# JiaoXianjun/multi-rtl-sdr-calibration

Hardware: AMD Instinct MI355X
Metric: IQ Msamples/s through FCCH+SCH calib (higher is better)
Workload: dtype f64; 1 GPU; cfg4 full chain gsm_sync_demod.m:107-124: 64 dongle streams (64/GPU) x 1020000 IQ samples (102 frames), fir1(46), FCCH+SCH+total_ppm_calculation, table on the host; streams_per_gpu=64, streams_total=64, output=table, collective=none, rows_checked_vs_oracle_per_rank=0

## Files before the change

multi-rtl-sdr-calibration_amd/csrc/kernels_detect.h:

```cpp
#pragma once
#include "state.h"
#include "kernels_frontend.h"

__device__ __forceinline__ constexpr int fft16_rev(int k) { return ((k & 1) << 3) | ((k & 2) << 1) | ((k & 4) >> 1) | ((k & 8) >> 3); }
__device__ __forceinline__ void fft16(cplx* x) {
    const double c1 = 0.92387953251128673848, s1 = 0.38268343236508978178;
    const double r2 = 0.70710678118654752440;
    const cplx w16[8] = {{1.0, 0.0}, {c1, -s1}, {r2, -r2}, {s1, -c1}, {0.0, -1.0}, {-s1, -c1}, {-r2, -r2}, {-c1, -s1}};
#pragma unroll
    for (int len = 16; len >= 2; len >>= 1) {
        const int half = len >> 1, step = 16 / len;
#pragma unroll
        for (int i = 0; i < 16; i += len) {
#pragma unroll
            for (int j = 0; j < half; ++j) {
                const cplx u = x[i + j], v = x[i + j + half];
                x[i + j] = make_double2(u.x + v.x, u.y + v.y);
                const cplx d = make_double2(u.x - v.x, u.y - v.y);
                const int t = j * step;
                if (t == 0) x[i + j + half] = d;
                else if (t == 4) x[i + j + half] = make_double2(d.y, -d.x);
                else x[i + j + half] = cmul(d, w16[t]);
            }
        }
// ... 1246 lines not shown
    __shared__ double sh_e[FK_THREADS / 64];
    __shared__ float sh_m[FK_THREADS / 64];
    __shared__ int sh_cnt;
    __shared__ double sh_D;
    const int tid = threadIdx.x;
    const int nstep = nshift - 1;
    const int nchunk = (nstep + FS_CHUNK - 1) / FS_CHUNK;
    const int total = *n_items;
    fft37_tables(w37, wN2, N2, tid, tw_g);
    DEV_STAMP(KID_CHUNK, blockIdx.x, 0);
    for (int it = blockIdx.x; it < total; it += gridDim.x) {
    const int item = items[it];
    const int c = item & 0xFF, widx = item >> 8, s = widx / H, w = widx - s * H;
    const double pstar = cert && cert[widx].p > 0.0 ? cert[widx].p : 0.0;
    const int t0 = c * FS_CHUNK;
    const int lim = nstep - t0 < FS_CHUNK ? nstep - t0 : FS_CHUNK;
    const cplx* x = win + (size_t)s * win_stream_stride + (size_t)w * win_stride + t0;
    __syncthreads();
    for (int i = tid; i < nfft + lim; i += FK_THREADS) xs[i] = x[i];
    if (tid == 0) sh_cnt = 0;
    __syncthreads();
    double e = 0.0;
    for (int i = tid; i < nfft; i += FK_THREADS) e += fabs(xs[i].x) + fabs(xs[i].y);
    if (tid < FS_CHUNK) {
        float2 v = make_float2(0.0f, 0.0f);
        double dabs = 0.0;
        if (tid < lim) {
            const cplx a1 = xs[tid + nfft], b1 = xs[tid];
            const double dr = a1.x - b1.x, di = a1.y - b1.y;
            v = make_float2((float)dr, (float)di);
            dabs = fabs(dr) + fabs(di);
            e += dabs;
        }
        d[tid] = v;
        dabs = wave_sum(dabs);
        if (tid == 0) sh_D = dabs;
    }
    for (int off = 32; off > 0; off >>= 1) e += __shfl_down(e, off, 64);
    if ((tid & 63) == 0) sh_e[tid >> 6] = e;
    __syncthreads();
    fft37_step1_sym(xs, B, w37, tw_g, nfft, N2, ldb, tid, FK_THREADS);
    __syncthreads();
    double es = 0.0;
    for (int i = 0; i < FK_THREADS / 64; ++i) es += sh_e[i];
    const double E = FS_ERR_SCALE_CHUNK * es;
    const int npair = nfft >> 1;
    const double sp = sqrt(pstar);
    ChunkRec* r = rec + ((size_t)s * H + w) * nchunk + c;
    float m = 0.0f;
    for (int g0 = 0; g0 < npair; g0 += FK_THREADS) {
        const int g = g0 + tid;
        const bool act = g < npair;
        const int jj = g / 37, kr = g - jj * 37;
        const int k0 = kr + 37 * jj, k1 = jj == 0 ? kr + 37 * (N2 >> 1) : kr + 37 * (N2 - jj);
        v2f best = {0.0f, 0.0f};
        if (act) {
            cplx X0, X1;
            fft37_step2_pair(B, wN2, N2, ldb, kr, jj, &X0, &X1);
            const cplx t0w = tw_g[k0], t1w = tw_g[k1];
            const v2f wr = {(float)t0w.x, (float)t1w.x}, wi = {(float)-t0w.y, (float)-t1w.y};
            v2f xr = {(float)X0.x, (float)X1.x}, xi = {(float)X0.y, (float)X1.y};
            if (c == 0) best = xr * xr + xi * xi;
            const double D = sh_D * (1.0 + 1e-9);
            const bool sweep = !(pstar > 0.0) || !((sqrt(X0.x * X0.x + X0.y * X0.y) + D) * (1.0 + 1e-9) < sp) ||
                               !((sqrt(X1.x * X1.x + X1.y * X1.y) + D) * (1.0 + 1e-9) < sp);
            if (sweep) {
#pragma unroll 8
            for (int t = 0; t < FS_CHUNK; ++t) {
                const float2 dv = d[t];
                const v2f dr = {dv.x, dv.x}, di = {dv.y, dv.y};
                const v2f ar = xr + dr, ai = xi + di;
                xr = ar * wr - ai * wi;
                xi = ar * wi + ai * wr;
                const v2f p = xr * xr + xi * xi;
                best.x = fmaxf(best.x, p.x);
                best.y = fmaxf(best.y, p.y);
            }
            }
            if (k1 == k0) best.y = 0.0f;
            m = fmaxf(m, fmaxf(best.x, best.y));
        }
        float mm = m;
        for (int off = 32; off > 0; off >>= 1) mm = fmaxf(mm, __shfl_xor(mm, off, 64));
        __syncthreads();
        if ((tid & 63) == 0) sh_m[tid >> 6] = mm;
        __syncthreads();
        float bm = sh_m[0];
        for (int i = 1; i < FK_THREADS / 64; ++i) bm = fmaxf(bm, sh_m[i]);
        double thr = sqrt((double)bm) - E;
        if (sp > thr) thr = sp;
        thr = (thr - E) * (1.0 - 1e-6);
        if (act && sqrt((double)best.x) >= thr) {
            const int i = atomicAdd(&sh_cnt, 1);
            if (i < FK_CAP) { r->cand[i].k = k0; r->cand[i].p = best.x; }
        }
        if (act && k1 != k0 && sqrt((double)best.y) >= thr) {
            const int i = atomicAdd(&sh_cnt, 1);
            if (i < FK_CAP) { r->cand[i].k = k1; r->cand[i].p = best.y; }
        }
    }
    __syncthreads();
    for (int off = 32; off > 0; off >>= 1) m = fmaxf(m, __shfl_xor(m, off, 64));
    if ((tid & 63) == 0) sh_m[tid >> 6] = m;
    __syncthreads();
    if (tid == 0) {
        float bm = sh_m[0];
        for (int i = 1; i < FK_THREADS / 64; ++i) bm = fmaxf(bm, sh_m[i]);
        r->amax = bm;
        r->E = E;
        r->count = sh_cnt <= FK_CAP ? sh_cnt : -1;
    }
    DEV_STAMP(KID_CHUNK, blockIdx.x, 1 + (it / gridDim.x < 6 ? it / gridDim.x : 6));
    }
}

__global__ void k_fine_openall(const StreamState* __restrict__ sts, int nchunk, int H, int* __restrict__ items,
                               int* __restrict__ n_items) {
    const int s = blockIdx.y, w = blockIdx.x;
    if (w >= sts[s].n_win) return;
    __shared__ int base;
    if (threadIdx.x == 0) base = atomicAdd(n_items, nchunk);
    __syncthreads();
    for (int c = threadIdx.x; c < nchunk; c += blockDim.x) items[base + c] = ((s * H + w) << 8) | c;
}

#define FV_MAX_ITEMS 512
#define FV_THREADS 256
__device__ __forceinline__ void peak_store(PeakOut* dst, const PeakOut& o) {
    static_assert(sizeof(PeakOut) == 16, "two 64-bit words");
    unsigned long long* d = (unsigned long long*)dst;
    __hip_atomic_store(d, (unsigned long long)__double_as_longlong(o.p), __ATOMIC_RELAXED, __HIP_MEMORY_SCOPE_AGENT);
    __hip_atomic_store(d + 1, (unsigned long long)(unsigned)o.tie | ((unsigned long long)(unsigned)o.k << 32), __ATOMIC_RELAXED,
                       __HIP_MEMORY_SCOPE_AGENT);
}
template <int FVT, int ANB = 19>
__device__ __forceinline__ void fine_verify_body(const StreamState* __restrict__ sts,
                                                 const cplx* __restrict__ win, long win_stream_stride,
                                                 long win_stride, int nshift, int nfft,
                                                 const cplx* __restrict__ tw_g, const ChunkRec* __restrict__ rec,
                                                 PeakOut* __restrict__ out, int H,
                                                 const FineCert* __restrict__ cert, int* __restrict__ n_open,
                                                 unsigned char* smem, PeakOut* res = nullptr) {
    if (blockIdx.x == 0 && blockIdx.y == 0 && threadIdx.x == 0) *n_open = 0;
    const int wlen = nshift - 1 + nfft;
    cplx* xs = (cplx*)smem;
    cplx* anchor = xs + wlen;
    int* items = (int*)(anchor + FV_MAX_ITEMS);
    __shared__ int n_items, n_over;
    __shared__ double red_p[FVT / 64];
    __shared__ int red_t[FVT / 64], red_k[FVT / 64];
    const int s = blockIdx.y, w = blockIdx.x;
    if (w >= sts[s].n_win) return;
    const int tid = threadIdx.x, lane = tid & 63, wave = tid >> 6;
    const int nstep = nshift - 1;
    const int nchunk = (nstep + FS_CHUNK - 1) / FS_CHUNK;
    FineCert fc;
    fc.p = -1.0; fc.t = 0x7fffffff; fc.k = 0x7fffffff; fc.nch = nchunk; fc.nsuf = 0;
    if (cert) {
        fc = cert[(size_t)s * H + w];
        if (fc.nch == 0) {
            if (tid == 0) { PeakOut o2; o2.p = fc.p; o2.tie = fc.t; o2.k = fc.k; if (res) *res = o2; else peak_store(&out[(size_t)s * H + w], o2); }
            return;
        }
    }
    const int nopen = fc.nch, nsuf = fc.nsuf;
    ChunkRec* r = (ChunkRec*)smem;
    {
        const uint4* src = (const uint4*)(rec + ((size_t)s * H + w) * nchunk);
        uint4* dst = (uint4*)r;
        constexpr int Q = (int)(sizeof(ChunkRec) / 16);
        for (int i = tid; i < nopen * Q; i += FVT) { const int j = i / Q; dst[i] = src[fc_open_chunk(j, nopen, nsuf, nchunk) * Q + (i - j * Q)]; }
    }
    if (tid == 0) { n_items = 0; n_over = 0; }
    __syncthreads();
    double L = fc.p > 0.0 ? sqrt(fc.p) : 0.0;
    for (int c = 0; c < nopen; ++c) {
        const double v = sqrt((double)r[c].amax) - r[c].E;
        if (v > L) L = v;
    }
    L *= 1.0 - 1e-9;
    for (int i = tid; i < nopen * FK_CAP; i += FVT) {
        const int c = i / FK_CAP, q = i - c * FK_CAP;
        const int cnt = r[c].count;
        if (cnt < 0) { if (q == 0) atomicAdd(&n_over, 1); continue; }
        if (q >= cnt) continue;
        const ChunkCand cc = r[c].cand[q];
        if (sqrt((double)cc.p) + r[c].E >= L) {
            const int idx = atomicAdd(&n_items, 1);
            if (idx < FV_MAX_ITEMS) items[idx] = (cc.k << 8) | fc_open_chunk(c, nopen, nsuf, nchunk);
        }
    }
    __syncthreads();
    const bool slow = n_over > 0 || n_items > FV_MAX_ITEMS;
    DEV_STAMP(KID_VERIFY, blockIdx.y * gridDim.x + blockIdx.x, 3);
    if (n_items == 0 && !slow && fc.p > 0.0) {
        if (tid == 0) { PeakOut o2; o2.p = fc.p; o2.tie = fc.t; o2.k = fc.k; if (res) *res = o2; else peak_store(&out[(size_t)s * H + w], o2); }
        return;
    }
    const cplx* x = win + (size_t)s * win_stream_stride + (size_t)w * win_stride;
    double best = -1.0;
    int bt = 0x7fffffff, bk = 0x7fffffff;
    if (tid == 0 && fc.p > 0.0) { best = fc.p; bt = fc.t; bk = fc.k; }
    if (n_items > 0 || slow) {
        for (int i = tid; i < wlen; i += FVT) xs[i] = x[i];
        __syncthreads();
        const long total = slow ? (long)nopen * nfft : (long)n_items;
        for (long base = 0; base < total; base += FV_MAX_ITEMS) {
            const int ni = (int)(total - base < FV_MAX_ITEMS ? total - base : FV_MAX_ITEMS);
            if (slow) {
                __syncthreads();
                for (int i = tid; i < ni; i += FVT) {
                    const long g = base + i;
                    items[i] = ((int)(g % nfft) << 8) | fc_open_chunk((int)(g / nfft), nopen, nsuf, nchunk);
                }
                __syncthreads();
            }
            for (int i = wave; i < ni; i += FVT / 64) {
                const int k = items[i] >> 8, c = items[i] & 0xFF;
                const int t0 = c * FS_CHUNK;
                const cplx av = anchor_dft<ANB>(xs + t0, k, tw_g, nfft, lane);
                const double a0r = av.x, a0i = av.y;
                const int lim = nstep - t0 < FS_CHUNK ? nstep - t0 : FS_CHUNK;
                double sr = 0.0, si = 0.0;
                if (lane < lim) {
                    const cplx xa = xs[t0 + lane + nfft], xb = xs[t0 + lane];
                    const cplx t = tw_g[((unsigned)k * (unsigned)lane) % (unsigned)nfft];
                    const double dr = xa.x - xb.x, di = xa.y - xb.y;
                    sr = dr * t.x - di * t.y;
                    si = dr * t.y + di * t.x;
                }
                sr = wave_scan_incl(sr);
                si = wave_scan_incl(si);
                if (lane < lim) {
                    const double xr = a0r + sr, xi = a0i + si;
                    const double p = xr * xr + xi * xi;
                    const int m = t0 + lane + 1;
                    if (p > best || (p == best && (m < bt || (m == bt && k < bk)))) { best = p; bt = m; bk = k; }
                }
                if (c == 0 && lane == 0) {
                    const double p = a0r * a0r + a0i * a0i;
                    if (p > best || (p == best && (0 < bt || (0 == bt && k < bk)))) { best = p; bt = 0; bk = k; }
                }
            }
        }
    }
    DEV_STAMP(KID_VERIFY, blockIdx.y * gridDim.x + blockIdx.x, 5);
#ifdef GSMCAL_DEVTIMING
    if (g_stamps && tid == 0 && blockIdx.y * gridDim.x + blockIdx.x < DEV_STAMP_BLOCKS) g_stamps[((size_t)KID_VERIFY * DEV_STAMP_BLOCKS + blockIdx.y * gridDim.x + blockIdx.x) * 16 + 15] = (unsigned long long)n_items * 100ull + (unsigned long long)nopen * 10000000ull;
#endif
    for (int off = 32; off > 0; off >>= 1) {
        const double op = __shfl_down(best, off, 64);
        const int ot = __shfl_down(bt, off, 64);
        const int ok = __shfl_down(bk, off, 64);
        if (op > best || (op == best && (ot < bt || (ot == bt && ok < bk)))) { best = op; bt = ot; bk = ok; }
    }
    if (lane == 0) { red_p[wave] = best; red_t[wave] = bt; red_k[wave] = bk; }
    __syncthreads();
    if (tid == 0) {
        for (int i = 1; i < FVT / 64; ++i)
            if (red_p[i] > best || (red_p[i] == best && (red_t[i] < bt || (red_t[i] == bt && red_k[i] < bk)))) {
                best = red_p[i]; bt = red_t[i]; bk = red_k[i];
            }
        PeakOut o2; o2.p = best; o2.tie = bt; o2.k = bk;
        if (res) *res = o2; else peak_store(&out[(size_t)s * H + w], o2);
    }
}

__device__ __forceinline__ float fc_group8_sum(float v) {
    int t;
    t = __builtin_amdgcn_update_dpp(0, __float_as_int(v), 0xB1, 0xF, 0xF, true);
    v += __int_as_float(t);
    t = __builtin_amdgcn_update_dpp(0, __float_as_int(v), 0x4E, 0xF, 0xF, true);
    v += __int_as_float(t);
    t = __builtin_amdgcn_update_dpp(0, __float_as_int(v), 0x141, 0xF, 0xF, true);
    v += __int_as_float(t);
    return v;
}

__host__ __device__ inline int fc_gcd64(int n) { int b = 64; while (n % b) b >>= 1; return b; }
__host__ __device__ constexpr int fc_threads(int nshift) {
    return ((nshift - 1) / FS_CHUNK * FC_NB + 63) / 64 * 64 < 256 ? 256 : ((nshift - 1) / FS_CHUNK * FC_NB + 63) / 64 * 64;
}
#define FC_XP(p) ((p) + ((p) >> 7))
struct FusedGather {
    const uint8_t* raw; long raw_stride;
    const double* coef;
    cplx* win_out;
    int ntaps, per;
    int sym47, pad;
};
__host__ inline size_t fc_stage_bytes(int per, int ntaps) {
    const int span8 = per + ntaps + 8;
    return (size_t)(span8 + span8 / 4 + 1) * sizeof(cplx) + (size_t)fir_taps_padded(ntaps) * sizeof(double);
}
__host__ inline size_t fc_lds_bytes(int nshift, int nfft) {
    const int nstep = nshift - 1, wlen = nstep + nfft, B = fc_gcd64(nfft);
    size_t r1 = (size_t)FC_NB * (wlen / B) * sizeof(cplx), e1 = (size_t)(nstep + 2) * sizeof(double);
    size_t r2 = (size_t)FC_NB * (B + 2 + nfft / B) * sizeof(cplx), e2 = (size_t)2 * (size_t)(FC_XP(nstep + 2) + 1) * sizeof(float) + 16 * sizeof(double);
    return (size_t)FC_XP(wlen) * sizeof(cplx) + (r1 > e1 ? r1 : e1) + (r2 > e2 ? r2 : e2);
}

#define FC_PRIO(P0, P1, P2) if (gridDim.x * gridDim.y <= 768u) { const unsigned rnd_ = (blockIdx.y * gridDim.x + blockIdx.x) >> 8; if (rnd_ == 0) __builtin_amdgcn_s_setprio(P0); else if (rnd_ == 1) __builtin_amdgcn_s_setprio(P1); else __builtin_amdgcn_s_setprio(P2); }
#define FC_PF 8
template <int OV, int NTAPS>
__global__ void __launch_bounds__(512) k_fine_cert(const StreamState* __restrict__ sts,
                                                   const cplx* __restrict__ win, long win_stream_stride,
                                                   long win_stride, int nshift_rt, int nfft_rt,
                                                   const cplx* __restrict__ tw_g, FineCert* __restrict__ cert, int H,
                                                   int* __restrict__ items, int* __restrict__ n_items, FusedGather fg_in) {
    extern __shared__ __attribute__((aligned(16))) unsigned char smem[];
    const int nshift = OV > 0 ? 128 * OV + 1 : nshift_rt, nfft = OV > 0 ? 148 * OV : nfft_rt;
    FusedGather fg = fg_in;
    if (OV > 0) fg.ntaps = NTAPS;
    const int nstep = nshift - 1, wlen = nstep + nfft;
    const int B = fc_gcd64(nfft), nA = nfft / B, nM = wlen / B, nchunk = nstep / FS_CHUNK;
    const int nthr = blockDim.x;
    cplx* xs = (cplx*)smem;
    const size_t r1 = (size_t)FC_NB * nM * sizeof(cplx), e1 = (size_t)(nstep + 2) * sizeof(double);
    cplx* Sp = xs + FC_XP(wlen);
    double* Et = (double*)Sp;
    unsigned char* reg2 = (unsigned char*)Sp + (r1 > e1 ? r1 : e1);
    const int ld1 = B + 2;
    cplx* tw1 = (cplx*)reg2;
    cplx* tw2 = tw1 + FC_NB * ld1;
    float* sumS = (float*)reg2;
    float* Cs = sumS + FC_XP(nstep + 2);
    double* sh_scan = (double*)(Cs + FC_XP(nstep + 2) + (FC_XP(nstep + 2) & 1));
    double* sh_scan2 = sh_scan + 8;
    __shared__ double red_p[8];
    __shared__ int red_t[8], red_k[8];
    __shared__ int sh_a, sh_b, sh_lo;
    const int s = blockIdx.y, w = blockIdx.x;
    if (w >= sts[s].n_win) return;
    const int tid = threadIdx.x, lane = tid & 63, wave = tid >> 6, nwave = nthr >> 6;
    DEV_STAMP(KID_CERT, blockIdx.y * gridDim.x + blockIdx.x, 0);
    FC_PRIO(0, 1, 2)
    if (fg.raw) {
        const StreamState* st = sts + s;
        const long n0 = st->n0, ws = st->win_start[w];
        const double mr = st->mean_re, mi = st->mean_im;
        const int ntp = fg.ntaps, per = fg.per;
        cplx* xq = (cplx*)Sp;
        double* c_s = (double*)(xq + xs_pad(per + ntp + 8) + 1);
        const unsigned short* base = (const unsigned short*)(fg.raw + (size_t)s * fg.raw_stride);
        cplx* wout = fg.win_out + (size_t)s * win_stream_stride + (size_t)w * win_stride;
        fir_stage_taps(c_s, fg.coef, ntp, tid, nthr);
        const bool sym47 = OV > 0 && NTAPS == 47 && fg.sym47 != 0;
        double cf[24];
        if (OV > 0 && NTAPS == 47) {
#pragma unroll
            for (int k = 0; k < 24; ++k) cf[k] = fg.coef[k];
        }
        const long ao = (long)(((uintptr_t)base >> 1) & 7);
        auto raw_chunk = [&](long first, int span, long& first_al) -> uint4 {
            long m = (first + ao) % 8;
            if (m < 0) m += 8;
            first_al = first - m;
            uint4 v = make_uint4(0, 0, 0, 0);
            const long g0 = first_al + 8L * tid;
            if (g0 < first + span) {
                if (g0 >= 0 && g0 + 8 <= n0) {
                    v = *(const uint4*)(base + g0);
                } else {
                    unsigned short t[8];
#pragma unroll
                    for (int i = 0; i < 8; ++i) t[i] = (g0 + i >= 0 && g0 + i < n0) ? base[g0 + i] : (unsigned short)0;
                    v.x = t[0] | ((unsigned)t[1] << 16); v.y = t[2] | ((unsigned)t[3] << 16);
                    v.z = t[4] | ((unsigned)t[5] << 16); v.w = t[6] | ((unsigned)t[7] << 16);
                }
            }
            return v;
        };
        long first_al;
        uint4 pre = raw_chunk(ws - (ntp - 1), (per < wlen ? per : wlen) + ntp - 1, first_al);
        for (int o0 = 0; o0 < wlen; o0 += per) {
            const int cnt = wlen - o0 < per ? wlen - o0 : per;
            const long first = ws + o0 - (ntp - 1);
            const int span = cnt + ntp - 1;
            {
                const int i_base = 8 * tid - (int)(first - first_al);
                const unsigned wv[4] = {pre.x, pre.y, pre.z, pre.w};
                const long g_base = first + i_base;
                if (i_base >= 0 && i_base + 8 <= span && g_base >= 0 && g_base + 8 <= n0) {
                    const int r = __builtin_amdgcn_readfirstlane(i_base & 3);
                    cplx* xp = xq + xs_pad(i_base);
#pragma unroll
                    for (int u = 0; u < 8; ++u) {
                        const unsigned q = wv[u >> 1] >> (16 * (u & 1));
                        xp[u + ((r + u) >> 2)] = make_double2((double)(q & 0xFFu) - mr, (double)((q >> 8) & 0xFFu) - mi);
                    }
                } else {
#pragma unroll
                    for (int u = 0; u < 8; ++u) {
                        const int i = i_base + u;
                        const long g = first + i;
                        const unsigned q = (wv[u >> 1] >> (16 * (u & 1))) & 0xFFFFu;
                        cplx v = make_double2(0.0, 0.0);
                        if (i < span && g >= 0 && g < n0) v = make_double2((double)(q & 0xFF) - mr, (double)(q >> 8) - mi);
                        if (i >= 0 && i < span + 8) xq[xs_pad(i)] = v;
                    }
                }
            }
            __syncthreads();
            if (o0 == 0) DEV_STAMP(KID_CERT, blockIdx.y * gridDim.x + blockIdx.x, 8);
            if (o0 + per < wlen) {
                const int ncnt = wlen - (o0 + per) < per ? wlen - (o0 + per) : per;
                pre = raw_chunk(first + per, ncnt + ntp - 1, first_al);
            }
            for (int i0 = 4 * tid; i0 < cnt; i0 += 4 * nthr) {
                cplx y0, y1, y2, y3;
                if (OV > 0 && NTAPS == 47 && sym47) {
                    cplx y[4];
                    fir4_sym47(xq, cf, i0, y);
                    y0 = y[0]; y1 = y[1]; y2 = y[2]; y3 = y[3];
                } else if (ntp == 47) fir4_lds<47>(xq, c_s, i0, ntp, &y0, &y1, &y2, &y3);
                else fir4_lds<0>(xq, c_s, i0, ntp, &y0, &y1, &y2, &y3);
                const int o = o0 + i0;
#ifdef GSMCAL_AB_LAZY_WIN
                xs[FC_XP(o)] = y0;
                if (i0 + 1 < cnt) xs[FC_XP(o + 1)] = y1;
                if (i0 + 2 < cnt) xs[FC_XP(o + 2)] = y2;
                if (i0 + 3 < cnt) xs[FC_XP(o + 3)] = y3;
#else
                xs[FC_XP(o)] = y0; wout[o] = y0;
                if (i0 + 1 < cnt) { xs[FC_XP(o + 1)] = y1; wout[o + 1] = y1; }
                if (i0 + 2 < cnt) { xs[FC_XP(o + 2)] = y2; wout[o + 2] = y2; }
                if (i0 + 3 < cnt) { xs[FC_XP(o + 3)] = y3; wout[o + 3] = y3; }
#endif
            }
            __syncthreads();
            DEV_STAMP(KID_CERT, blockIdx.y * gridDim.x + blockIdx.x, 9 + (o0 > 0) + (o0 > per));
        }
        if (tid == 0) { sh_a = 0; sh_b = nstep; }
        __syncthreads();
    } else {
        const cplx* x = win + (size_t)s * win_stream_stride + (size_t)w * win_stride;
        for (int i = tid; i < wlen; i += nthr) xs[FC_XP(i)] = x[i];
        if (tid == 0) { sh_a = 0; sh_b = nstep; }
        __syncthreads();
    }
    DEV_STAMP(KID_CERT, blockIdx.y * gridDim.x + blockIdx.x, 1);
    FC_PRIO(2, 1, 0)
    {
        const int D = nfft / 148, n0 = nstep / 2;
        cplx* yd = Sp;
        cplx* t148 = Sp + 148;
        double* pw = (double*)(Sp + 296);
        for (int m = tid; m < 148; m += nthr) {
            double sr = 0.0, si = 0.0;
            for (int i = 0; i < D; ++i) { const cplx v = xs[FC_XP(n0 + D * m + i)]; sr += v.x; si += v.y; }
            yd[m] = make_double2(sr, si);
            t148[m] = tw_g[D * m];
        }
        __syncthreads();
        cplx* A = (cplx*)(pw + 148);
        for (int o = tid; o < 148; o += nthr) {
            const int n2 = o / 37, k1 = o - n2 * 37;
            double ar = 0.0, ai = 0.0;
            int idx = 0;
#pragma unroll 4
            for (int n1 = 0; n1 < 37; ++n1) {
                const cplx v = yd[4 * n1 + n2], t = t148[idx];
                ar = fma(v.x, t.x, fma(-v.y, t.y, ar));
                ai = fma(v.x, t.y, fma(v.y, t.x, ai));
                idx += 4 * k1;
                idx = idx >= 148 ? idx - 148 : idx;
            }
            A[o] = make_double2(ar, ai);
        }
        __syncthreads();
        for (int q = tid; q < 148; q += nthr) {
            const int k1 = q % 37;
            double ar = 0.0, ai = 0.0;
            int idx = 0;
#pragma unroll
            for (int n2 = 0; n2 < 4; ++n2) {
                const cplx v = A[n2 * 37 + k1], t = t148[idx];
                ar = fma(v.x, t.x, fma(-v.y, t.y, ar));
                ai = fma(v.x, t.y, fma(v.y, t.x, ai));
                idx += q;
                idx = idx >= 148 ? idx - 148 : idx;
            }
            pw[q] = ar * ar + ai * ai;
        }
        __syncthreads();
        if (wave == 0) {
            double bp = -1.0;
            int bq = 0;
            for (int q = lane; q < 148; q += 64)
                if (pw[q] > bp) { bp = pw[q]; bq = q; }
            for (int off = 32; off > 0; off >>= 1) {
                const double op = __shfl_down(bp, off, 64);
                const int oq = __shfl_down(bq, off, 64);
                if (op > bp || (op == bp && oq < bq)) { bp = op; bq = oq; }
            }
            if (lane == 0) {
                const bool up = pw[(bq + 1) % 148] > pw[(bq + 147) % 148];
                const int kpk = bq < 74 ? bq : nfft - 148 + bq;
                sh_lo = kpk - (up ? FC_NB / 2 - 1 : FC_NB / 2);
            }
        }
        __syncthreads();
    }
    const int lo = sh_lo;
    DEV_STAMP(KID_CERT, blockIdx.y * gridDim.x + blockIdx.x, 2);
    const int j = tid & (FC_NB - 1), c = tid / FC_NB;
    const bool act = c < nchunk;
    const int k = ((lo + j) % nfft + nfft) % nfft;
    for (int i = tid; i < FC_NB * (B + nA); i += nthr) {
        if (i < FC_NB * B) {
            const int jj = i / B, q = i - jj * B;
            const int kk = ((lo + jj) % nfft + nfft) % nfft;
            tw1[jj * ld1 + q] = tw_g[(kk * q) % nfft];
        } else {
            const int ii = i - FC_NB * B;
            const int q = ii / FC_NB, jj = ii - q * FC_NB;
            const int kk = ((lo + jj) % nfft + nfft) % nfft;
            tw2[q * FC_NB + jj] = tw_g[(((kk * B) % nfft) * q) % nfft];
        }
    }
    __syncthreads();
    for (int m = c; m < nM; m += nthr / FC_NB) {
        const int xb0 = B * m;
        const unsigned char* xp = (const unsigned char*)(xs + FC_XP(xb0));
        const unsigned char* tp = (const unsigned char*)(tw1 + j * ld1);
        const unsigned wrap = (unsigned)B * (unsigned)sizeof(cplx) - 1u;
        unsigned o = (unsigned)(c & (B - 1)) * (unsigned)sizeof(cplx);
        double ar = 0.0, ai = 0.0;
#pragma unroll 4
        for (int i = 0; i < B; ++i) {
            const cplx v = *(const cplx*)(xp + o), t = *(const cplx*)(tp + o);
            ar = fma(v.x, t.x, fma(-v.y, t.y, ar));
            ai = fma(v.x, t.y, fma(v.y, t.x, ai));
            o = (o + (unsigned)sizeof(cplx)) & wrap;
        }
        Sp[j * nM + m] = make_double2(ar, ai);
    }
    __syncthreads();
    DEV_STAMP(KID_CERT, blockIdx.y * gridDim.x + blockIdx.x, 3);
    double xr = 0.0, xi = 0.0;
    if (act) {
        const cplx* sb = Sp + j * nM + (FS_CHUNK / B) * c;
        const cplx* tb = tw2 + j;
#pragma unroll 4
        for (int a = 0; a < nA; ++a) {
            const cplx v = sb[a], t = tb[a * FC_NB];
            xr = fma(v.x, t.x, fma(-v.y, t.y, xr));
            xi = fma(v.x, t.y, fma(v.y, t.x, xi));
        }
    }
    __syncthreads();
    DEV_STAMP(KID_CERT, blockIdx.y * gridDim.x + blockIdx.x, 4);
    FC_PRIO(0, 1, 2)
    {
        double e0 = 0.0;
        for (int i = tid; i < nfft; i += nthr) { const cplx v = xs[FC_XP(i)]; e0 += v.x * v.x + v.y * v.y; }
        for (int off = 32; off > 0; off >>= 1) e0 += __shfl_down(e0, off, 64);
        if (lane == 0) red_p[wave] = e0;
        const int per = (nstep + nthr - 1) / nthr;
        const int i0 = tid * per < nstep ? tid * per : nstep, i1 = i0 + per < nstep ? i0 + per : nstep;
        double loc = 0.0, locd = 0.0;
        for (int q = i0; q < i1; ++q) {
            const cplx a1 = xs[FC_XP(q + nfft)], b1 = xs[FC_XP(q)];
            loc += (a1.x * a1.x + a1.y * a1.y) - (b1.x * b1.x + b1.y * b1.y);
            const double dr = a1.x - b1.x, di = a1.y - b1.y;
            locd += (double)(__fsqrt_rn((float)(dr * dr + di * di)) * 1.00000095367431640625f);
        }
        double inc = loc, incd = locd;
        for (int off = 1; off < 64; off <<= 1) {
            const double o = __shfl_up(inc, off, 64), od = __shfl_up(incd, off, 64);
            if (lane >= off) { inc += o; incd += od; }
        }
        if (lane == 63) { sh_scan[wave] = inc; sh_scan2[wave] = incd; }
        __syncthreads();
        double run = inc - loc, rund = incd - locd;
        for (int i = 0; i < wave; ++i) { run += sh_scan[i]; rund += sh_scan2[i]; }
        for (int i = 0; i < nwave; ++i) run += red_p[i];
        for (int q = i0; q < i1; ++q) {
            Et[q] = run;
            Cs[FC_XP(q)] = (float)rund;
            const cplx a1 = xs[FC_XP(q + nfft)], b1 = xs[FC_XP(q)];
            run += (a1.x * a1.x + a1.y * a1.y) - (b1.x * b1.x + b1.y * b1.y);
            const double dr = a1.x - b1.x, di = a1.y - b1.y;
            rund += (double)(__fsqrt_rn((float)(dr * dr + di * di)) * 1.00000095367431640625f);
        }
        if (i1 == nstep && i0 < nstep) { Et[nstep] = run; Cs[FC_XP(nstep)] = (float)rund; }
    }
    DEV_STAMP(KID_CERT, blockIdx.y * gridDim.x + blockIdx.x, 5);
    double best = -1.0;
    int bt = 0x7fffffff;
    if (act) {
        const cplx wk = tw_g[k];
        const double wr = wk.x, wi = -wk.y;
        const int t0 = c * FS_CHUNK;
        if (c == 0) {
            const double p = xr * xr + xi * xi;
            best = p; bt = 0;
            sumS[FC_XP(0)] = fc_group8_sum((float)p);
        }
        const int xa0 = t0 + nfft, xb0 = t0;
        for (int q0 = 0; q0 < FS_CHUNK; q0 += FC_PF) {
            double dr[FC_PF], di[FC_PF];
#pragma unroll
            for (int u = 0; u < FC_PF; ++u) {
                const cplx a1 = xs[FC_XP(xa0 + q0 + u)], b1 = xs[FC_XP(xb0 + q0 + u)];
                dr[u] = a1.x - b1.x;
                di[u] = a1.y - b1.y;
            }
            float ps[FC_PF];
#pragma unroll
            for (int u = 0; u < FC_PF; ++u) {
                const double ar = xr + dr[u], ai = xi + di[u];
                xr = ar * wr - ai * wi;
                xi = ar * wi + ai * wr;
                const double p = xr * xr + xi * xi;
                if (p > best) { best = p; bt = t0 + q0 + u + 1; }
                ps[u] = fc_group8_sum((float)p);
            }
#pragma unroll
            for (int u = 0; u < FC_PF; ++u) sumS[FC_XP(t0 + q0 + u + 1)] = ps[u];
        }
    }
    int bk = k;
    for (int off = 32; off > 0; off >>= 1) {
        const double op = __shfl_down(best, off, 64);
        const int ot = __shfl_down(bt, off, 64);
        const int ok = __shfl_down(bk, off, 64);
        if (op > best || (op == best && (ot < bt || (ot == bt && ok < bk)))) { best = op; bt = ot; bk = ok; }
    }
    __syncthreads();
    DEV_STAMP(KID_CERT, blockIdx.y * gridDim.x + blockIdx.x, 6);
    if (lane == 0) { red_p[wave] = best; red_t[wave] = bt; red_k[wave] = bk; }
    __syncthreads();
    best = red_p[0]; bt = red_t[0]; bk = red_k[0];
    for (int i = 1; i < nwave; ++i)
        if (red_p[i] > best || (red_p[i] == best && (red_t[i] < bt || (red_t[i] == bt && red_k[i] < bk)))) {
            best = red_p[i]; bt = red_t[i]; bk = red_k[i];
        }
    {
        const double INF = __longlong_as_double(0x7ff0000000000000LL);
        const double sb = best > 0.0 ? sqrt(best) * (1.0 - 1e-9) : -1.0;
        const int per = (nstep + nthr) / nthr;
        const int u0 = tid * per < nstep + 1 ? tid * per : nstep + 1, u1 = u0 + per < nstep + 1 ? u0 + per : nstep + 1;
        double mf = INF, mb = INF;
        for (int t = u0; t < u1; ++t) {
            const double NE = (double)nfft * Et[t];
            const float ss = sumS[FC_XP(t)];
            const double R = NE - (double)ss + 4e-6 * NE;
            float sf = ss <= 3.0e38f ? __fsqrt_rn((float)(R > 0.0 ? R : 0.0)) * 1.000001f : __int_as_float(0x7f800000);
            if (!(sf >= 0.0f)) sf = __int_as_float(0x7f800000);
            const double sv = (double)sf;
            (void)sv;
            sumS[FC_XP(t)] = sf;
            const double cv = (double)Cs[FC_XP(t)];
            mf = fmin(mf, (double)sf - cv);
            mb = fmin(mb, (double)sf + cv);
        }
        double pf = mf, pb = mb;
        for (int off = 1; off < 64; off <<= 1) {
            const double o = __shfl_up(pf, off, 64), ob = __shfl_down(pb, off, 64);
            if (lane >= off) pf = fmin(pf, o);
            if (lane + off < 64) pb = fmin(pb, ob);
        }
        __syncthreads();
        if (lane == 63) sh_scan[wave] = pf;
        if (lane == 0) sh_scan2[wave] = pb;
        double ef = __shfl_up(pf, 1, 64), eb = __shfl_down(pb, 1, 64);
        if (lane == 0) ef = INF;
        if (lane == 63) eb = INF;
        __syncthreads();
        for (int i = 0; i < wave; ++i) ef = fmin(ef, sh_scan[i]);
        for (int i = wave + 1; i < nwave; ++i) eb = fmin(eb, sh_scan2[i]);
        const double ctot = (double)Cs[FC_XP(nstep)] * 1e-6;
        unsigned okm = 0;
        for (int t = u0; t < u1; ++t) {
            const double cv = (double)Cs[FC_XP(t)];
            ef = fmin(ef, (double)sumS[FC_XP(t)] - cv);
            if (cv + ef + ctot < sb) okm |= 1u << (t - u0);
        }
        for (int t = u1 - 1; t >= u0; --t) {
            const double cv = (double)Cs[FC_XP(t)];
            eb = fmin(eb, (double)sumS[FC_XP(t)] + cv);
            const bool okc = ((okm >> (t - u0)) & 1u) || (eb - cv + ctot < sb);
            if (!okc) {
                if (t <= bt) atomicMax(&sh_a, t + 1);
                if (t >= bt) atomicMin(&sh_b, t - 1);
            }
        }
    }
    __syncthreads();
#ifdef GSMCAL_AB_LAZY_WIN
    if (fg.raw && OV > 0 && NTAPS == 47 && fg.sym47 != 0 && (sh_a != 0 || sh_b < nstep)) {
        cplx* wout = fg.win_out + (size_t)s * win_stream_stride + (size_t)w * win_stride;
        for (int i = tid; i < wlen; i += nthr) wout[i] = xs[FC_XP(i)];
    }
#endif
    if (tid == 0) {
        FineCert o;
        o.p = best; o.t = bt; o.k = bk; o.a = sh_a; o.b = sh_b;
        const int a = sh_a, b = sh_b;
        int npre = a == 0 ? 0 : (a == 1 ? 1 : (a - 2) / FS_CHUNK + 1);
        int nsuf = b < nstep ? nchunk - b / FS_CHUNK : 0;
        if (npre + nsuf > nchunk) { npre = nchunk; nsuf = 0; }
        o.nch = npre + nsuf; o.nsuf = nsuf;
        cert[(size_t)s * H + w] = o;
        if (o.nch > 0) {
            const int base = atomicAdd(n_items, o.nch);
            for (int i = 0; i < o.nch; ++i) items[base + i] = ((s * H + w) << 8) | fc_open_chunk(i, o.nch, nsuf, nchunk);
        }
    }
    DEV_STAMP(KID_CERT, blockIdx.y * gridDim.x + blockIdx.x, 7);
}

__global__ void __launch_bounds__(256) k_fine_search(const StreamState* __restrict__ sts,
                                                     const cplx* __restrict__ win, long win_stream_stride,
                                                     long win_stride, int nshift, int nfft,
                                                     const cplx* __restrict__ x0, PeakOut* __restrict__ out,
                                                     int H, int NB) {
    extern __shared__ __attribute__((aligned(16))) unsigned char smem[];
    cplx* d = (cplx*)smem;
    __shared__ double red_p[4];
    __shared__ int red_t[4], red_k[4];
    const int s = blockIdx.z, w = blockIdx.y;
    if (w >= sts[s].n_win) return;
    const cplx* x = win + (size_t)s * win_stream_stride + (size_t)w * win_stride;
    const int tid = threadIdx.x;
    const int nstep = nshift - 1;
    const int nstep_pad = (nstep + FS_CHUNK - 1) / FS_CHUNK * FS_CHUNK;
    const int k = blockIdx.x * 256 + tid;
    const bool cand = k < nfft;
    for (int t = tid; t < nstep_pad; t += 256) {
        cplx v = make_double2(0.0, 0.0);
        if (t < nstep) {
            const cplx a = x[t + nfft], b = x[t];
            v = make_double2(a.x - b.x, a.y - b.y);
        }
        d[t] = v;
    }
    __syncthreads();
    double best = -1.0;
    int best_c = -1;
    double sxr = 0.0, sxi = 0.0;
    double wr = 1.0, wi = 0.0;
    if (cand) {
        sincospi(2.0 * (double)k / (double)nfft, &wi, &wr);
        const cplx xi0 = x0[((size_t)s * H + w) * nfft + k];
        double xr = xi0.x, xi = xi0.y;
        best = xr * xr + xi * xi;
        const int nchunk = nstep_pad / FS_CHUNK;
        for (int c = 0; c < nchunk; ++c) {
            const double cxr = xr, cxi = xi;
            double cmax = -1.0;
            const cplx* dc = d + c * FS_CHUNK;
            const int lim = nstep - c * FS_CHUNK;
            if (lim >= FS_CHUNK) {
#pragma unroll 8
                for (int j = 0; j < FS_CHUNK; ++j) {
                    const cplx dv = dc[j];
                    const double ar = xr + dv.x, ai = xi + dv.y;
                    xr = ar * wr - ai * wi;
                    xi = ar * wi + ai * wr;
                    cmax = fmax(cmax, xr * xr + xi * xi);
                }
            } else {
                for (int j = 0; j < lim; ++j) {
                    const cplx dv = dc[j];
                    const double ar = xr + dv.x, ai = xi + dv.y;
                    xr = ar * wr - ai * wi;
                    xi = ar * wi + ai * wr;
                    cmax = fmax(cmax, xr * xr + xi * xi);
                }
            }
            if (cmax > best) { best = cmax; best_c = c; sxr = cxr; sxi = cxi; }
        }
    }
    double rb = best;
    int rc = cand ? best_c : 0x7ffffff0, rk = k;
    for (int off = 32; off > 0; off >>= 1) {
        const double op = __shfl_down(rb, off, 64);
        const int oc = __shfl_down(rc, off, 64);
        const int ok = __shfl_down(rk, off, 64);
        if (op > rb || (op == rb && (oc < rc || (oc == rc && ok < rk)))) { rb = op; rc = oc; rk = ok; }
    }
    const int wv = tid >> 6;
    if ((tid & 63) == 0) { red_p[wv] = rb; red_t[wv] = rc; red_k[wv] = rk; }
    __syncthreads();
    rb = red_p[0]; rc = red_t[0]; rk = red_k[0];
    for (int i = 1; i < 4; ++i)
        if (red_p[i] > rb || (red_p[i] == rb && (red_t[i] < rc || (red_t[i] == rc && red_k[i] < rk)))) {
            rb = red_p[i]; rc = red_t[i]; rk = red_k[i];
        }
    if (k == rk) {
        int m = 0;
        if (best_c >= 0) {
            double xr = sxr, xi = sxi;
            const cplx* dc = d + best_c * FS_CHUNK;
            const int lim = nstep - best_c * FS_CHUNK < FS_CHUNK ? nstep - best_c * FS_CHUNK : FS_CHUNK;
            for (int j = 0; j < lim; ++j) {
                const cplx dv = dc[j];
                const double ar = xr + dv.x, ai = xi + dv.y;
                xr = ar * wr - ai * wi;
                xi = ar * wi + ai * wr;
                const double p = xr * xr + xi * xi;
                if (p == best) { m = best_c * FS_CHUNK + j + 1; break; }
            }
        }
        PeakOut o; o.p = best; o.tie = m; o.k = k;
        out[((size_t)s * H + w) * NB + blockIdx.x] = o;
    }
}
```

Before: 560,200 Msample/s.

## Warp-specialize energy prefix scans onto idle waves in fine-cert kernel

Result: faster. 566,400 Msample/s, median of 6 (+1.1%).

```diff
diff --git a/multi-rtl-sdr-calibration_amd/csrc/kernels_detect.h b/multi-rtl-sdr-calibration_amd/csrc/kernels_detect.h
--- a/multi-rtl-sdr-calibration_amd/csrc/kernels_detect.h
+++ b/multi-rtl-sdr-calibration_amd/csrc/kernels_detect.h
@@ -1572,6 +1572,15 @@
 
 #define FC_PRIO(P0, P1, P2) if (gridDim.x * gridDim.y <= 768u) { const unsigned rnd_ = (blockIdx.y * gridDim.x + blockIdx.x) >> 8; if (rnd_ == 0) __builtin_amdgcn_s_setprio(P0); else if (rnd_ == 1) __builtin_amdgcn_s_setprio(P1); else __builtin_amdgcn_s_setprio(P2); }
 #define FC_PF 8
+#ifdef GSMCAL_DEVTIMING
+#define FC_ROLE_STAMP(wv, i)                                                                                          \
+    do {                                                                                                              \
+        if (DEV_STAMP_ON(KID_CERT, i) && g_stamps && wave == (wv) && lane == 0 && blockIdx.y * gridDim.x + blockIdx.x < DEV_STAMP_BLOCKS) \
+            g_stamps[((size_t)KID_CERT * DEV_STAMP_BLOCKS + blockIdx.y * gridDim.x + blockIdx.x) * 16 + (i)] = wall_clock64();           \
+    } while (0)
+#else
+#define FC_ROLE_STAMP(wv, i) do { } while (0)
+#endif
 template <int OV, int NTAPS>
 __global__ void __launch_bounds__(512) k_fine_cert(const StreamState* __restrict__ sts,
                                                    const cplx* __restrict__ win, long win_stream_stride,
@@ -1822,7 +1831,57 @@
     __syncthreads();
     DEV_STAMP(KID_CERT, blockIdx.y * gridDim.x + blockIdx.x, 4);
     FC_PRIO(0, 1, 2)
-    {
+    const int nslide = (FC_NB * nchunk + 63) >> 6;
+    const bool split = nwave - nslide >= 2;
+    if (split) {
+        DEV_STAMP(KID_CERT, blockIdx.y * gridDim.x + blockIdx.x, 5);
+        if (wave == nslide || wave == nslide + 1) {
+            const bool we = wave == nslide;
+            const int per = OV > 0 ? 2 * OV : (nstep + 63) >> 6;
+            const int i0 = lane * per < nstep ? lane * per : nstep, i1 = i0 + per < nstep ? i0 + per : nstep;
+            auto term = [&](int q) -> double {
+                const cplx a1 = xs[FC_XP(q + nfft)], b1 = xs[FC_XP(q)];
+                if (we) return (a1.x * a1.x + a1.y * a1.y) - (b1.x * b1.x + b1.y * b1.y);
+                const double dr = a1.x - b1.x, di = a1.y - b1.y;
+                return (double)(__fsqrt_rn((float)(dr * dr + di * di)) * 1.00000095367431640625f);
+            };
+            double run = 0.0;
+            if (we) {
+                for (int i = lane; i < nfft; i += 64) { const cplx v = xs[FC_XP(i)]; run += v.x * v.x + v.y * v.y; }
+                for (int off = 32; off > 0; off >>= 1) run += __shfl_down(run, off, 64);
+                run = __shfl(run, 0, 64);
+            }
+            double g[OV > 0 ? 2 * OV : 1];
+            double loc = 0.0;
+            if (OV > 0) {
+#pragma unroll
+                for (int u = 0; u < 2 * OV; ++u) { g[u] = term(i0 + u); loc += g[u]; }
+            } else {
+                for (int q = i0; q < i1; ++q) loc += term(q);
+            }
+            double inc = loc;
+            for (int off = 1; off < 64; off <<= 1) {
+                const double o = __shfl_up(inc, off, 64);
+                if (lane >= off) inc += o;
+            }
+            const double exc = __shfl_up(inc, 1, 64);
+            if (lane > 0) run += exc;
+            if (OV > 0) {
+#pragma unroll
+                for (int u = 0; u < 2 * OV; ++u) {
+                    if (we) Et[i0 + u] = run; else Cs[FC_XP(i0 + u)] = (float)run;
+                    run += g[u];
+                }
+            } else {
+                for (int q = i0; q < i1; ++q) {
+                    if (we) Et[q] = run; else Cs[FC_XP(q)] = (float)run;
+                    run += term(q);
+                }
+            }
+            if (i1 == nstep && i0 < nstep) { if (we) Et[nstep] = run; else Cs[FC_XP(nstep)] = (float)run; }
+            FC_ROLE_STAMP(wave, we ? 12 : 13);
+        }
+    } else {
         double e0 = 0.0;
         for (int i = tid; i < nfft; i += nthr) { const cplx v = xs[FC_XP(i)]; e0 += v.x * v.x + v.y * v.y; }
         for (int off = 32; off > 0; off >>= 1) e0 += __shfl_down(e0, off, 64);
@@ -1855,8 +1914,8 @@
             rund += (double)(__fsqrt_rn((float)(dr * dr + di * di)) * 1.00000095367431640625f);
         }
         if (i1 == nstep && i0 < nstep) { Et[nstep] = run; Cs[FC_XP(nstep)] = (float)rund; }
-    }
-    DEV_STAMP(KID_CERT, blockIdx.y * gridDim.x + blockIdx.x, 5);
+        DEV_STAMP(KID_CERT, blockIdx.y * gridDim.x + blockIdx.x, 5);
+    }
     double best = -1.0;
     int bt = 0x7fffffff;
     if (act) {
@@ -1891,6 +1950,7 @@
             for (int u = 0; u < FC_PF; ++u) sumS[FC_XP(t0 + q0 + u + 1)] = ps[u];
         }
     }
+    FC_ROLE_STAMP(0, 14);
     int bk = k;
     for (int off = 32; off > 0; off >>= 1) {
         const double op = __shfl_down(best, off, 64);
```
